# arkworks-rs/pcd

Measured on AMD Instinct MI355X. Metric: msm_mscalar_mul_per_s, higher is better.
Workload: dtype u32 (11 x 28-bit unsaturated Montgomery limbs, v_mad_u64_u32 with 64-bit column accumulators); 1 GPU; MNT4-298 G1 variable-base MSM, n=1048576 pairs per GPU (2^20 per GPU), proving-key bases and scalars resident in HBM, scalar distribution uniform; curve=MNT4-298, group=G1, log_n=20, window_bits=20, windows=15

## Files before the change

pcd_amd/csrc/msm.hip.h:

```cpp
#pragma once
#include <cstdlib>
#include <math.h>

#include <algorithm>
#include <type_traits>
#include <vector>

#include "ec.hip.h"

namespace pcd {

template <int K>
struct EventSet {
  hipEvent_t e[K] = {};
  bool live = false;
  hipError_t create() {
    for (int i = 0; i < K; i++) { hipError_t r = hipEventCreate(&e[i]); if (r != hipSuccess) return r; }
    live = true;
    return hipSuccess;
  }
  hipEvent_t operator[](int i) const { return e[i]; }
  ~EventSet() { for (int i = 0; i < K; i++) if (e[i]) (void)hipEventDestroy(e[i]); }
};

// ... 254 lines not shown
  off[(size_t)b * KB + 2 * t] = ex;
  off[(size_t)b * KB + 2 * t + 1] = ex + c0;
  __syncthreads();
  for (uint32_t p0 = lo + threadIdx.x; p0 < hi; p0 += MSM_SORT_UNROLL * blockDim.x) {
    uint64_t e[MSM_SORT_UNROLL];
    uint32_t pos[MSM_SORT_UNROLL];
#pragma unroll
    for (int u = 0; u < MSM_SORT_UNROLL; u++) { uint32_t p = p0 + u * blockDim.x; e[u] = p < hi ? entries[p] : ~0ull; }
#pragma unroll
    for (int u = 0; u < MSM_SORT_UNROLL; u++) if (e[u] != ~0ull) pos[u] = atomicAdd(&hist[(uint32_t)(e[u] >> 32) & (KB - 1)], 1u);
#pragma unroll
    for (int u = 0; u < MSM_SORT_UNROLL; u++) if (e[u] != ~0ull) sorted_idx[pos[u]] = (uint32_t)e[u];
  }
}

static __global__ void __launch_bounds__(1024) scan_block_sums(const uint32_t* __restrict__ in, uint32_t n, uint32_t per_block,
                                                         uint32_t* __restrict__ block_sums) {
  __shared__ uint32_t sh[1024];
  uint32_t b = blockIdx.x, lo = b * per_block, hi = min(n, lo + per_block);
  uint32_t acc = 0;
  for (uint32_t i = lo + threadIdx.x; i < hi; i += blockDim.x) acc += in[i];
  sh[threadIdx.x] = acc;
  __syncthreads();
  for (int s = 512; s > 0; s >>= 1) { if ((int)threadIdx.x < s) sh[threadIdx.x] += sh[threadIdx.x + s]; __syncthreads(); }
  if (threadIdx.x == 0) block_sums[b] = sh[0];
}
static __global__ void __launch_bounds__(1024) scan_apply(const uint32_t* __restrict__ in, uint32_t n, uint32_t per_block,
                                                    const uint32_t* __restrict__ block_sums, uint32_t nblocks,
                                                    uint32_t* __restrict__ out ) {
  __shared__ uint32_t sh[1024];
  __shared__ uint32_t carry;
  uint32_t b = blockIdx.x, lo = b * per_block, hi = min(n, lo + per_block);
  if (threadIdx.x == 0) { uint32_t a = 0; for (uint32_t k = 0; k < b; k++) a += block_sums[k]; carry = a; }
  __syncthreads();
  for (uint32_t base = lo; base < hi; base += 1024) {
    uint32_t i = base + threadIdx.x;
    uint32_t v = (i < hi) ? in[i] : 0;
    sh[threadIdx.x] = v;
    __syncthreads();
    for (int s = 1; s < 1024; s <<= 1) {
      uint32_t t = ((int)threadIdx.x >= s) ? sh[threadIdx.x - s] : 0;
      __syncthreads();
      sh[threadIdx.x] += t;
      __syncthreads();
    }
    if (i < hi) out[i] = carry + sh[threadIdx.x] - v;
    __syncthreads();
    if (threadIdx.x == 0) carry += sh[1023];
    __syncthreads();
  }
  if (b == nblocks - 1 && threadIdx.x == 0) out[n] = carry;
}

PCD_HD uint32_t msm_plan_chunk(uint32_t M, uint32_t lanes, uint32_t lo, uint32_t hi) {
  const uint64_t per_round = (uint64_t)lanes * hi;
  const uint64_t rounds = ((uint64_t)M + per_round - 1) / per_round;
  const uint32_t chunk = rounds ? (uint32_t)(((uint64_t)M + (uint64_t)lanes * rounds - 1) / ((uint64_t)lanes * rounds)) : lo;
  return chunk < lo ? lo : chunk > hi ? hi : chunk;
}
PCD_HD uint32_t msm_plan_word(uint32_t lanes, uint32_t lo, uint32_t hi) { return lanes | (lo << 20) | (hi << 26); }
PCD_HD uint32_t msm_chunk_of_plan(uint32_t M, uint32_t plan) { return msm_plan_chunk(M, plan & 0xFFFFFu, (plan >> 20) & 63u, (plan >> 26) & 63u); }

PCD_DEV uint32_t msm_find_key(const uint32_t* __restrict__ off, uint32_t nkeys, uint32_t p) {
  uint32_t lo = 0, hi = nkeys;
  while (hi - lo > 1) { uint32_t mid = (lo + hi) >> 1; if (off[mid] <= p) lo = mid; else hi = mid; }
  return lo;
}

struct MsmEntrySource {
  const uint32_t* sorted_idx;
  const uint32_t* slots;
  const uint32_t* ones_idx;
  const uint32_t* flag;
  uint32_t cap, ones_key;
};
struct MsmCursor {
  uint32_t key, key_start, key_end;
  uint32_t next_end;
  PCD_DEV void seek(const uint32_t* __restrict__ off, uint32_t nkeys, uint32_t p) {
    key = msm_find_key(off, nkeys, p);
    key_start = off[key];
    key_end = off[key + 1];
    next_end = key + 2 <= nkeys ? off[key + 2] : key_end;
  }
  PCD_DEV void advance_to(const uint32_t* __restrict__ off, uint32_t nkeys, uint32_t p) {
    for (int step = 0; step < 4 && p >= key_end; step++) {
      key++; key_start = key_end; key_end = next_end;
      next_end = key + 2 <= nkeys ? off[key + 2] : key_end;
    }
    if (p >= key_end) seek(off, nkeys, p);
  }
};
PCD_DEV uint32_t msm_entry(const MsmEntrySource& src, bool compact, const MsmCursor& cur, uint32_t p) {
  if (cur.key == src.ones_key) return compact && !src.ones_idx ? src.sorted_idx[p] : src.ones_idx[p - cur.key_start];
  return compact ? src.sorted_idx[p] : src.slots[(size_t)cur.key * src.cap + (p - cur.key_start)];
}

#ifndef PCD_BASE_ALIGN
#define PCD_BASE_ALIGN 1
#endif
template <class G>
struct MsmBaseStride {
  static constexpr int W = Aff<typename G::F>::WORDS;
  static constexpr int value = (PCD_BASE_ALIGN && W == 22) ? 32 : W;
};

template <class G>
struct MsmUseXyzz {
  typedef typename G::F F;
#ifndef PCD_XYZZ_753
#define PCD_XYZZ_753 0
#endif
  static constexpr bool value = F::Base::INLINE_ARITH || F::DEG == 2 || (PCD_XYZZ_753 && F::Base::N > 11);
};
// ... 89 lines not shown
    typename EC<G>::AccX a = {F::load(p), F::load(p + F::WORDS), F::load(p + 2 * F::WORDS), F::load(p + 3 * F::WORDS)};
    return EC<G>::x_to_jac(a);
  }
  static constexpr bool SEPARATE = true;
};
template <class G>
struct MsmStoredPlain<G, false> {
  typedef typename G::F F;
  static constexpr int WORDS = Jac<F>::WORDS;
  PCD_DEV static Jac<F> load(const uint32_t* p) { return Jac<F>::load(p); }
  static constexpr bool SEPARATE = false;
};
template <class G, bool LAZY = LazyCapable<typename G::F>::value>
struct MsmStored : MsmStoredPlain<G> {};
template <class G>
struct MsmStored<G, true> {
  typedef typename G::F F;
  static constexpr int WORDS = EC<G>::ACC_WORDS;
  PCD_DEV static Jac<F> load(const uint32_t* p) {
    typename EC<G>::AccLz a;
    a.ZZ = F::load(p + 2 * F::WORDS);
    if (a.ZZ.is_zero()) return Jac<F>::infinity();
    a.inf = false;
#pragma unroll
    for (int i = 0; i < F::N; i++) a.X.v[i] = (int32_t)p[i];
    a.Y = F::load(p + F::WORDS);
    a.ZZZ = F::load(p + 3 * F::WORDS);
    return EC<G>::lz_to_jac(a);
  }
  static constexpr bool SEPARATE = true;
};

template <class G>
struct MsmAccWaves {
  typedef typename AccOf<G>::type::F FA;
#ifndef PCD_ACC_WAVES_SPLIT
#define PCD_ACC_WAVES_SPLIT 2
#endif
#ifndef PCD_ACC_WAVES_G1
#define PCD_ACC_WAVES_G1 2
#endif
#ifndef PCD_ACC_WAVES_MB298
#define PCD_ACC_WAVES_MB298 2
#endif
  static constexpr int value = !FA::Base::INLINE_ARITH ? (FA::Base::N <= 11 ? PCD_ACC_WAVES_MB298 : 1)
                             : FA::DEG == 1 ? PCD_ACC_WAVES_G1 : AccOf<G>::LANES > 1 ? PCD_ACC_WAVES_SPLIT : 1;
};

template <class G, bool COMPACT>
__global__ void __launch_bounds__(64, MsmAccWaves<G>::value) msm_accumulate_kernel(const uint32_t* __restrict__ bases, const MsmEntrySource src,
                                                            const uint32_t* __restrict__ off, uint32_t nkeys,
                                                            uint32_t chunk, uint32_t* __restrict__ buckets,
                                                            uint32_t* __restrict__ piece_first, uint32_t* __restrict__ piece_last,
                                                            uint32_t plan ) {
  if (plan) chunk = msm_chunk_of_plan(off[nkeys], plan);
  typedef typename AccOf<G>::type GA;
  typedef typename GA::F F;
  typedef EC<GA> E;
  constexpr int RW = MsmStored<GA>::WORDS;
  constexpr uint32_t LANES = AccOf<G>::LANES, PER_WAVE = 64 / LANES;
  if (threadIdx.x >= PER_WAVE * LANES) return;
  uint32_t t = blockIdx.x * PER_WAVE + threadIdx.x / LANES;
  const uint32_t M = off[nkeys];
  uint64_t start64 = (uint64_t)t * chunk;
  if (start64 >= M) return;
  uint32_t start = (uint32_t)start64, end = (uint32_t)min((uint64_t)M, start64 + chunk);
  if (!COMPACT && src.flag && *src.flag != 0) return;
  if (COMPACT && src.flag && *src.flag == 0) return;
  MsmCursor cur;
  cur.seek(off, nkeys, start);
  bool open_start = cur.key_start < start;
#if PCD_ACC_LDS
  typename std::conditional<LazyCapable<F>::value, MsmRunLazyLds<GA>, MsmRunPlain<GA>>::type acc;
#else
  typename std::conditional<LazyCapable<F>::value, MsmRunLazy<GA>, MsmRunPlain<GA>>::type acc;
#endif
  constexpr bool PREFETCH = F::Base::INLINE_ARITH;
  const uint32_t ones_start = off[src.ones_key];
  auto point_of = [&](uint32_t e) {
    Aff<F> q = Aff<F>::load(bases + (size_t)(e & ~MSM_NEG) * MsmBaseStride<G>::value);
    const F ny = q.y.neg();
    if (e & MSM_NEG) q.y = ny;
    return q;
  };
  if constexpr (COMPACT) {
    auto entry_at = [&](uint32_t pos) { return (src.ones_idx && pos >= ones_start) ? src.ones_idx[pos - ones_start] : src.sorted_idx[pos]; };
    Aff<F> nxt;
    if (PREFETCH) nxt = point_of(entry_at(start));
    for (uint32_t p = start; p < end; p++) {
      if (p >= cur.key_end) {
        if (open_start) { acc.flush(piece_first + (size_t)t * RW); open_start = false; }
        else acc.flush(buckets + (size_t)cur.key * RW);
        cur.advance_to(off, nkeys, p);
      }
      if (PREFETCH) {
        const Aff<F> pt = nxt;
        if (p + 1 < end) nxt = point_of(entry_at(p + 1));
        acc.add(pt);
      } else {
        acc.add(point_of(entry_at(p)));
      }
    }
  } else {
    MsmCursor nxt_cur = cur;
    Aff<F> nxt;
    if (PREFETCH) nxt = point_of(msm_entry(src, false, cur, start));
    for (uint32_t p = start; p < end; p++) {
// ... 259 lines not shown
      MsmRunPlain<GA> acc;
      uint32_t key = key_first;
      for (uint32_t i = 0; i < cnt; i++) {
        const uint32_t k0 = in[(size_t)(2 * i) * 64], l0 = in[(size_t)(2 * i + 1) * 64];
        if (k0 != key) {
          if (open_start) { acc.flush(piece_first + (size_t)t * RW); open_start = false; }
          else acc.flush(buckets + (size_t)key * RW);
          key = k0;
        }
        acc.add(point_of(l0));
      }
      const bool open_end = off[key + 1] > end;
      if (open_end) acc.flush(piece_last + (size_t)t * RW);
      else if (open_start) acc.flush(piece_first + (size_t)t * RW);
      else acc.flush(buckets + (size_t)key * RW);
    }
  }
}

template <class G>
struct MsmItems {
  typedef typename SplitOfTail<G>::type GA;
  static constexpr uint32_t LANES = SplitOfTail<G>::LANES, PER_WAVE = 64 / LANES;
  PCD_DEV static bool idle() { return threadIdx.x >= PER_WAVE * LANES; }
  PCD_DEV static uint32_t local() { return threadIdx.x / LANES; }
  PCD_DEV static uint32_t item() { return blockIdx.x * PER_WAVE + threadIdx.x / LANES; }
  static uint32_t grid(uint32_t items) { return (items + PER_WAVE - 1) / PER_WAVE; }
};

static __global__ void __launch_bounds__(256) msm_zero_kernel(uint32_t* __restrict__ cnt, uint32_t n_cnt, uint32_t* __restrict__ ctl4) {
  const uint32_t i = blockIdx.x * blockDim.x + threadIdx.x;
  if (i < n_cnt) cnt[i] = 0;
  if (i < 4) ctl4[i] = 0;
}

#ifndef PCD_SINGLE_ITEM_PLAIN
#define PCD_SINGLE_ITEM_PLAIN 0
#endif
template <class G> struct MsmSingleItem {
  typedef typename std::conditional<PCD_SINGLE_ITEM_PLAIN != 0, typename SplitOf<G>::type, typename SplitOfTail<G>::type>::type GA;
  static constexpr int LANES = PCD_SINGLE_ITEM_PLAIN != 0 ? SplitOf<G>::LANES : SplitOfTail<G>::LANES;
};
template <class G>
__global__ void __launch_bounds__(64) msm_merge_ones_kernel(uint32_t* __restrict__ buckets, uint32_t ones_key) {
  typedef typename MsmSingleItem<G>::GA GA;
  typedef typename GA::F F;
  if (blockIdx.x != 0 || threadIdx.x >= MsmSingleItem<G>::LANES) return;
  Jac<F> a = Jac<F>::load(buckets + (size_t)1 * Jac<F>::WORDS);
  Jac<F> b = Jac<F>::load(buckets + (size_t)ones_key * Jac<F>::WORDS);
  EC<GA>::add(a, b).store(buckets + (size_t)1 * Jac<F>::WORDS);
}

template <class G>
__global__ void __launch_bounds__(64) msm_fixup_kernel(const uint32_t* __restrict__ off, uint32_t nkeys, uint32_t chunk,
                                                       const uint32_t* __restrict__ piece_first, const uint32_t* __restrict__ piece_last,
                                                       const uint32_t* __restrict__ acc_buckets ,
                                                       uint32_t* __restrict__ buckets, uint32_t big_limit, uint32_t* __restrict__ big_count,
                                                       uint32_t* __restrict__ big_list , uint32_t big_cap,
                                                       uint32_t* __restrict__ seg_list , uint32_t seg_len,
                                                       const uint32_t* __restrict__ chunk_dev ,
                                                       uint32_t plan ) {
  if (chunk_dev) chunk = *chunk_dev;
  else if (plan) chunk = msm_chunk_of_plan(off[nkeys], plan);
  typedef typename MsmItems<G>::GA GA;
  typedef typename GA::F F;
  typedef EC<GA> E;
  constexpr int RW = MsmStored<GA>::WORDS;
  if (MsmItems<G>::idle()) return;
  const bool lead = threadIdx.x % MsmItems<G>::LANES == 0;
  uint32_t key = MsmItems<G>::item();
  if (key >= nkeys) return;
  uint32_t lo = off[key], hi = off[key + 1];
  if (hi == lo) {
    F::zero().store(buckets + (size_t)key * Jac<F>::WORDS + 2 * F::WORDS);
    return;
  }
  uint32_t t0 = lo / chunk, t1 = (hi - 1) / chunk;
  if (t1 == t0) {
    if (MsmStored<GA>::SEPARATE) MsmStored<GA>::load(acc_buckets + (size_t)key * RW).store(buckets + (size_t)key * Jac<F>::WORDS);
    return;
  }
  if (t1 - t0 + 1 > big_limit) {
    if (!lead) return;
    uint32_t nseg = (t1 - t0 + seg_len) / seg_len;
    uint32_t slot = atomicAdd(&big_count[0], 1u);
    uint32_t s0 = atomicAdd(&big_count[1], nseg);
    if (slot < big_cap) { big_list[3 * slot] = key; big_list[3 * slot + 1] = s0; big_list[3 * slot + 2] = nseg; }
    for (uint32_t i = 0; i < nseg; i++) {
      uint32_t lo = t0 + i * seg_len, hi = min(t1, lo + seg_len - 1);
      seg_list[3 * (s0 + i)] = lo; seg_list[3 * (s0 + i) + 1] = hi; seg_list[3 * (s0 + i) + 2] = t1;
    }
    return;
  }
  Jac<F> acc = MsmStored<GA>::load(piece_last + (size_t)t0 * RW);
  for (uint32_t u = t0 + 1; u < t1; u++) acc = E::add(acc, MsmStored<GA>::load(piece_last + (size_t)u * RW));
  acc = E::add(acc, MsmStored<GA>::load(piece_first + (size_t)t1 * RW));
  acc.store(buckets + (size_t)key * Jac<F>::WORDS);
}

template <class G, bool ENABLE = true, bool Q = true>
struct MsmPairItems {
  static constexpr bool TWO = ENABLE && TwoLaneOps<G>::value && (MsmItems<G>::LANES == 1 || HalfLanes<typename MsmItems<G>::GA::F>::L == (int)MsmItems<G>::LANES);
  static constexpr bool QUAD = Q && TWO && MsmItems<G>::LANES == 1 && PCD_EC4 != 0;
  static constexpr uint32_t BASE = MsmItems<G>::LANES, LANES = QUAD ? 4 : TWO ? 2 * BASE : BASE, PER_WAVE = 64 / LANES;
  PCD_DEV static bool idle() { return threadIdx.x >= PER_WAVE * LANES; }
  PCD_DEV static uint32_t item() { return blockIdx.x * PER_WAVE + threadIdx.x / LANES; }
  PCD_DEV static uint32_t local() { return threadIdx.x / LANES; }
  PCD_DEV static bool writer() { return QUAD ? (threadIdx.x & 3u) == 0 : (!TWO || (((threadIdx.x & 63u) / BASE) & 1u) == 0); }
  static uint32_t grid(uint32_t items) { return (items + PER_WAVE - 1) / PER_WAVE; }
};
template <class G, bool TWO = MsmPairItems<G, true>::TWO, bool Q = true>
struct MsmPairOps {
  typedef typename MsmItems<G>::GA GA;
  typedef Jac<typename GA::F> J;
  PCD_DEV static J add(const J& a, const J& b) { return EC<GA>::add(a, b); }
  PCD_DEV static J dbl(const J& a) { return EC<GA>::dbl(a); }
};
template <class G, bool Q>
struct MsmPairOps<G, true, Q> {
  typedef typename SplitOfTail<G>::type GA;
  typedef Jac<typename GA::F> J;
  PCD_DEV static J add(const J& a, const J& b) { if constexpr (MsmPairItems<G, true, Q>::QUAD) return EC4<GA>::add4(a, b); else return EC2<GA>::add2(a, b); }
  PCD_DEV static J dbl(const J& a) { if constexpr (MsmPairItems<G, true, Q>::QUAD) return EC4<GA>::dbl4(a); else return EC2<GA>::dbl2(a); }
};
template <class G>
PCD_DEV void msm_wave_tree(Jac<typename MsmPairOps<G>::GA::F> acc, uint32_t* my , uint32_t* dst) {
  typedef MsmPairItems<G> IT;
  typedef MsmPairOps<G> O;
  typedef typename O::GA::F F;
  constexpr uint32_t PW = IT::PER_WAVE;
  const uint32_t it = IT::local();
  const bool live = !IT::idle();
  if (live && IT::writer()) acc.store(my + (size_t)it * Jac<F>::WORDS);
  __syncthreads();
  for (uint32_t s = 32; s > 0; s >>= 1) {
    if (live && it < s && it + s < PW) {
      Jac<F> o = Jac<F>::load(my + (size_t)(it + s) * Jac<F>::WORDS);
      acc = O::add(acc, o);
      if (IT::writer()) acc.store(my + (size_t)it * Jac<F>::WORDS);
    }
    __syncthreads();
  }
  if (live && it == 0 && IT::writer()) acc.store(dst);
  __syncthreads();
}
template <class G>
__global__ void __launch_bounds__(64) msm_big_segments_kernel(const uint32_t* __restrict__ seg_list, const uint32_t* __restrict__ big_count,
                                                              const uint32_t* __restrict__ piece_first, const uint32_t* __restrict__ piece_last,
                                                              uint32_t* __restrict__ partial, uint32_t* __restrict__ scratch) {
  typedef MsmPairItems<G> IT;
  typedef MsmPairOps<G> O;
  typedef typename O::GA GA;
  typedef typename GA::F F;
  constexpr uint32_t PW = IT::PER_WAVE;
  const uint32_t nseg = big_count[1];
  uint32_t* my = scratch + (size_t)blockIdx.x * 64 * Jac<F>::WORDS;
  for (uint32_t sg = blockIdx.x; sg < nseg; sg += gridDim.x) {
    uint32_t lo = seg_list[3 * sg], hi = seg_list[3 * sg + 1], tlast = seg_list[3 * sg + 2];
    Jac<F> acc = Jac<F>::infinity();
    if (!IT::idle())
      for (uint32_t u = lo + IT::local(); u <= hi; u += PW) {
        const uint32_t* src = (u == tlast) ? piece_first : piece_last;
        acc = O::add(acc, MsmStored<GA>::load(src + (size_t)u * MsmStored<GA>::WORDS));
      }
    msm_wave_tree<G>(acc, my, partial + (size_t)sg * Jac<F>::WORDS);
  }
}
template <class G>
__global__ void __launch_bounds__(64) msm_big_bucket_kernel(const uint32_t* __restrict__ big_list, const uint32_t* __restrict__ big_count,
                                                            const uint32_t* __restrict__ partial, uint32_t* __restrict__ buckets,
                                                            uint32_t* __restrict__ scratch) {
  typedef MsmPairItems<G> IT;
  typedef MsmPairOps<G> O;
  typedef typename O::GA GA;
  typedef typename GA::F F;
  constexpr uint32_t PW = IT::PER_WAVE;
  const uint32_t nbig = big_count[0];
  uint32_t* my = scratch + (size_t)blockIdx.x * 64 * Jac<F>::WORDS;
  for (uint32_t b = blockIdx.x; b < nbig; b += gridDim.x) {
    uint32_t key = big_list[3 * b], s0 = big_list[3 * b + 1], ns = big_list[3 * b + 2];
    Jac<F> acc = Jac<F>::infinity();
    if (!IT::idle())
      for (uint32_t u = IT::local(); u < ns; u += PW) acc = O::add(acc, Jac<F>::load(partial + (size_t)(s0 + u) * Jac<F>::WORDS));
    msm_wave_tree<G>(acc, my, buckets + (size_t)key * Jac<F>::WORDS);
  }
}

template <class G, bool WIDE>
__global__ void __launch_bounds__(64) msm_tail_level_kernel(const uint32_t* __restrict__ A_in, uint32_t mA, size_t strideA_in,
                                                            const uint32_t* __restrict__ C_in, uint32_t mC, size_t strideC_in,
                                                            uint32_t* __restrict__ A_out, size_t strideA_out,
                                                            uint32_t* __restrict__ C_out, size_t strideC_out, int k) {
  typedef MsmPairItems<G, WIDE> IT;
  typedef MsmPairOps<G, IT::TWO> O;
  typedef typename O::GA GA;
  typedef typename GA::F F;
  constexpr int PW = Jac<F>::WORDS;
  if (IT::idle()) return;
  uint32_t K = 1u << k;
  uint32_t JA = (mA + K - 1) >> k, JC = (mC + K - 1) >> k;
  uint32_t tid = IT::item();
  uint32_t w = blockIdx.y;
  if (tid < JA) {
    const uint32_t* A = A_in + w * strideA_in * PW;
    Jac<F> run = Jac<F>::infinity(), acc = Jac<F>::infinity();
    for (int tt = (int)K - 1; tt >= 0; tt--) {
      uint32_t i = tid * K + tt;
      if (i < mA) run = O::add(run, Jac<F>::load(A + (size_t)i * PW));
      acc = O::add(acc, run);
    }
    if (IT::writer()) acc.store(C_out + (w * strideC_out + JC + tid) * PW);
    if (tid >= 1) {
      for (int d = 0; d < k; d++) run = O::dbl(run);
      if (IT::writer()) run.store(A_out + (w * strideA_out + tid - 1) * PW);
    }
  } else if (tid < JA + JC) {
    uint32_t j = tid - JA;
    const uint32_t* Cw = C_in + w * strideC_in * PW;
    Jac<F> acc = Jac<F>::infinity();
    for (uint32_t tt = 0; tt < K; tt++) {
      uint32_t i = j * K + tt;
      if (i < mC) acc = O::add(acc, Jac<F>::load(Cw + (size_t)i * PW));
    }
    if (IT::writer()) acc.store(C_out + (w * strideC_out + j) * PW);
  }
}

template <class G, bool Q = true>
PCD_DEV void msm_tail_pair_item(int role, uint32_t j, uint32_t w, const uint32_t* A_in, uint32_t mA, size_t strideA_in, const uint32_t* C_in,
                                uint32_t mC, size_t strideC_in, uint32_t* A_out, size_t strideA_out, uint32_t* C_out, size_t strideC_out) {
  typedef MsmPairOps<G, MsmPairItems<G, true>::TWO, Q> O;
  typedef typename O::GA GA;
  typedef typename GA::F F;
  typedef MsmPairItems<G, true, Q> IT;
  constexpr int PW = Jac<F>::WORDS;
  const uint32_t JA = (mA + 1) >> 1, JC = (mC + 1) >> 1;
  if (role < 2) {
    if (j >= JA) return;
    const uint32_t* A = A_in + w * strideA_in * PW;
    const bool two = 2 * j + 1 < mA;
    const Jac<F> a0 = Jac<F>::load(A + (size_t)(2 * j) * PW);
    if (role == 0) {
      if (j == 0) return;
      Jac<F> run = two ? O::add(a0, Jac<F>::load(A + (size_t)(2 * j + 1) * PW)) : a0;
      run = O::dbl(run);
      if (IT::writer()) run.store(A_out + (w * strideA_out + j - 1) * PW);
    } else {
      Jac<F> acc = two ? O::add(O::dbl(Jac<F>::load(A + (size_t)(2 * j + 1) * PW)), a0) : a0;
      if (IT::writer()) acc.store(C_out + (w * strideC_out + JC + j) * PW);
    }
  } else {
    if (j >= JC) return;
    const uint32_t* Cw = C_in + w * strideC_in * PW;
    Jac<F> acc = Jac<F>::load(Cw + (size_t)(2 * j) * PW);
    if (2 * j + 1 < mC) acc = O::add(acc, Jac<F>::load(Cw + (size_t)(2 * j + 1) * PW));
    if (IT::writer()) acc.store(C_out + (w * strideC_out + j) * PW);
  }
}
template <class G, bool Q = true>
__global__ void __launch_bounds__(64) msm_tail_pair_kernel(const uint32_t* __restrict__ A_in, uint32_t mA, size_t strideA_in,
                                                           const uint32_t* __restrict__ C_in, uint32_t mC, size_t strideC_in,
                                                           uint32_t* __restrict__ A_out, size_t strideA_out,
                                                           uint32_t* __restrict__ C_out, size_t strideC_out) {
  typedef MsmPairItems<G, true, Q> IT;
  if (IT::idle()) return;
  msm_tail_pair_item<G, Q>((int)blockIdx.z, IT::item(), blockIdx.y, A_in, mA, strideA_in, C_in, mC, strideC_in, A_out, strideA_out, C_out, strideC_out);
}
constexpr uint32_t MSM_FUSED_WAVES = 4;
#ifndef PCD_QUAD_MAX_ITEMS
#define PCD_QUAD_MAX_ITEMS 4096
#endif
constexpr uint32_t MSM_QUAD_MAX_ITEMS = PCD_QUAD_MAX_ITEMS;
template <class G>
struct MsmFusedTail {
  static constexpr bool ENABLED = !MsmPairOps<G>::GA::F::Base::MAILBOX;
  static uint32_t waves(uint32_t items) { return (items + MsmPairItems<G>::PER_WAVE - 1) / MsmPairItems<G>::PER_WAVE; }
  static bool fits(uint32_t mA, uint32_t mC) { return ENABLED && 2 * waves((mA + 1) >> 1) + waves((mC + 1) >> 1) <= MSM_FUSED_WAVES; }
};
template <class G>
__global__ void __launch_bounds__(64 * MSM_FUSED_WAVES) msm_tail_fused_kernel(const uint32_t* A_in, uint32_t mA, size_t strideA_in, const uint32_t* C_in,
                                                                              uint32_t mC, size_t strideC_in, uint32_t* A0, uint32_t* A1, uint32_t* C0,
                                                                              uint32_t* C1, size_t strideAC, int flip) {
  typedef MsmPairItems<G> IT;
  const uint32_t wave = threadIdx.x >> 6, lane = threadIdx.x & 63u;
  const bool idle = lane >= IT::PER_WAVE * IT::LANES;
  const uint32_t w = blockIdx.x;
  while (mA > 0 || mC > 1) {
    const uint32_t JA = (mA + 1) >> 1, JC = (mC + 1) >> 1;
    uint32_t* A_out = flip ? A1 : A0;
    uint32_t* C_out = flip ? C1 : C0;
    const uint32_t wa = (JA + IT::PER_WAVE - 1) / IT::PER_WAVE;
    const int role = wave < wa ? 0 : wave < 2 * wa ? 1 : 2;
    const uint32_t j = (wave - (uint32_t)role * wa) * IT::PER_WAVE + lane / IT::LANES;
    if (!idle) msm_tail_pair_item<G>(role, j, w, A_in, mA, strideA_in, C_in, mC, strideC_in, A_out, strideAC, C_out, strideAC);
    __syncthreads();
    mA = JA ? JA - 1 : 0;
    mC = JC + JA;
    A_in = A_out; strideA_in = strideAC;
    C_in = C_out; strideC_in = strideAC;
    flip ^= 1;
  }
}

template <class G>
__global__ void __launch_bounds__(64) msm_horner_kernel(const uint32_t* __restrict__ C, size_t strideC, int W, int c, uint32_t* __restrict__ out) {
  typedef typename MsmSingleItem<G>::GA GA;
  typedef typename GA::F F;
  typedef EC<GA> E;
  constexpr int PW = Jac<F>::WORDS;
  if (blockIdx.x != 0 || threadIdx.x >= MsmSingleItem<G>::LANES) return;
  Jac<F> total = Jac<F>::load(C + (size_t)(W - 1) * strideC * PW);
  for (int w = W - 2; w >= 0; w--) {
    for (int d = 0; d < c; d++) total = E::dbl(total);
    total = E::add(total, Jac<F>::load(C + (size_t)w * strideC * PW));
  }
  total.store(out);
}

template <class G>
// ... 123 lines not shown
struct MsmSharedSort {
  bool valid = false;
  uint32_t n = 0, n_total = 0, offset = 0, tkeys = 0;
  int c = 0, W = 0, groups = 0;
  const uint32_t* scalars = nullptr;
  const uint32_t* inf_bits = nullptr;
  MsmEntrySource src{};
  const uint32_t* off = nullptr;
  hipEvent_t ready = nullptr;
};
enum { MSM_SHARE_NONE = 0, MSM_SHARE_PRODUCE = 1, MSM_SHARE_CONSUME = 2 };

template <class G>
hipError_t msm_run(MsmWorkspace& ws, hipStream_t st, const MsmBasesView& bv, const uint32_t* scalars_dev, uint32_t n,
                   uint32_t* out_dev, int c_override, uint32_t chunk_override, int sort_mode, MsmTimings* tm,
                   MsmSharedSort* share = nullptr, int share_role = MSM_SHARE_NONE) {
  const int acc_mode = (sort_mode >> 4) & 3;
  const uint32_t tree_chunk = ((uint32_t)sort_mode >> 8) & 0xFFFu, tree_min_pairs = ((uint32_t)sort_mode >> 20) & 0xFFu;
  sort_mode &= 15;
  const bool single_pass = sort_mode == 1;
  const uint32_t* bases_dev = bv.dptr;
  typedef typename G::F F;
  constexpr int NS = G::FR::N32;
  constexpr int PW = Jac<F>::WORDS;
  constexpr size_t PB = (size_t)PW * 4;
  if (n == 0) { ws.last_err_dev = nullptr; Jac<F> inf = Jac<F>::infinity(); return hipMemcpyAsync(out_dev, &inf, PB, hipMemcpyHostToDevice, st); }
  MsmPlan pl;
  pl.n = n;
  pl.c = bv.groups > 1 ? bv.c : (c_override ? c_override : msm_pick_window(n, G::FR::BITS, 0));
  pl.W = msm_num_windows(G::FR::BITS, pl.c);
  const int Wg = (pl.W + bv.groups - 1) / bv.groups;
  pl.nkeys = (uint32_t)Wg << pl.c;
  const uint64_t maxM = (uint64_t)n * pl.W;
  pl.chunk = chunk_override ? chunk_override : 40;
  int& cus = ws.cus;
  if (!cus) {
    int dev = 0;
    if (hipGetDevice(&dev) != hipSuccess || hipDeviceGetAttribute(&cus, hipDeviceAttributeMultiprocessorCount, dev) != hipSuccess || cus <= 0) cus = 256;
  }
  bool use_tree = false;
  uint32_t tree_cap = 0;
  const uint32_t* tree_chunk_dev = nullptr;
  if constexpr (MsmTreeCapable<G>::value) {
    use_tree = acc_mode == 2 && (uint64_t)bv.n_total * bv.groups < MSM_SCR;
    if (use_tree) {
      tree_cap = tree_chunk ? tree_chunk : MSM_TREE_CHUNK_MAX;
      pl.chunk = tree_cap;
    }
  }
  const MsmLane* lane = ws.lane;
  const int plan_cus = lane && lane->cus > 0 ? lane->cus : cus;
  uint32_t acc_lanes = 0, chunk_lo = 0;
  static const uint32_t chunk_hi_env = getenv("PCDHIP_CHUNK_HI") ? (uint32_t)atoi(getenv("PCDHIP_CHUNK_HI")) : 0u;
  const uint32_t chunk_hi = chunk_hi_env >= 16 && chunk_hi_env <= 63 ? chunk_hi_env : 56;
  if (!chunk_override && !use_tree) {
    acc_lanes = (uint32_t)plan_cus * 4 * MsmAccWaves<G>::value * (64 / AccOf<G>::LANES);
    chunk_lo = (uint32_t)std::min<uint64_t>(40, std::max<uint64_t>(16, (maxM + 4ull * acc_lanes - 1) / (4ull * acc_lanes)));
    pl.chunk = chunk_lo;
  }
  const uint32_t plan_word = acc_lanes && acc_lanes < (1u << 20) && chunk_hi < 64 ? msm_plan_word(acc_lanes, chunk_lo, chunk_hi) : 0u;
  if (acc_lanes && !plan_word) pl.chunk = 40;
  if (maxM >= 0xFFFFFFF0ull || (uint64_t)bv.n_total * bv.groups >= 0x7FFFFFF0ull) return hipErrorInvalidValue;

  EventSet<9> ev;
  if (tm) PCD_HIP_TRY(ev.create());
  auto mark = [&](int i) -> hipError_t { return tm ? hipEventRecord(ev[i], st) : hipSuccess; };

  const uint32_t tkeys = pl.nkeys + 1, ones_key = pl.nkeys;
  const bool consume = share && share_role == MSM_SHARE_CONSUME && share->valid && share->n == n && share->n_total == bv.n_total &&
                       share->offset == bv.offset && share->tkeys == tkeys && share->c == pl.c && share->W == pl.W &&
                       share->groups == bv.groups && share->scalars == scalars_dev &&
                       (share->inf_bits == nullptr || share->inf_bits == bv.inf_bits);
  PCD_HIP_TRY(ws.ensure(WS_CNT, (size_t)tkeys * 4 + 16));
  PCD_HIP_TRY(ws.ensure(WS_OFF, ((size_t)tkeys + 1) * 4));
  const uint32_t scan_per_block = 16384;
  const uint32_t scan_blocks = (tkeys + scan_per_block - 1) / scan_per_block;
  PCD_HIP_TRY(ws.ensure(WS_BSUM, (size_t)scan_blocks * 4));
  PCD_HIP_TRY(ws.ensure(WS_SORTED, (size_t)maxM * 4));
  PCD_HIP_TRY(ws.ensure(WS_BUCKETS, (size_t)tkeys * PB));
  PCD_HIP_TRY(ws.ensure(WS_OUT, PB + 64));
  PCD_HIP_TRY(ws.ensure(WS_ONES, (size_t)n * 4 + 32));
  uint32_t* cnt = (uint32_t*)ws.buf[WS_CNT];
  uint32_t* off = (uint32_t*)ws.buf[WS_OFF];
  uint32_t* bsum = (uint32_t*)ws.buf[WS_BSUM];
  uint32_t* sorted = (uint32_t*)ws.buf[WS_SORTED];
  uint32_t* buckets = (uint32_t*)ws.buf[WS_BUCKETS];
  uint32_t* ones_idx = (uint32_t*)ws.buf[WS_ONES];
  uint32_t* flag = ones_idx + n;
  uint32_t* err = flag + 1;
  uint32_t* big_count = flag + 2;
  auto zero_start = [&](uint32_t n_cnt) {
    hipLaunchKernelGGL(msm_zero_kernel, dim3(std::max<uint32_t>(1u, (n_cnt + 255) / 256)), dim3(256), 0, st, cnt, n_cnt, flag);
  };
  ws.last_err_dev = consume ? nullptr : err;
  constexpr int SBITS = G::FR::BITS;
  const int wins = (pl.W + Wg - 1) / Wg;
  const int top_bits = G::FR::BITS + 1 - (pl.W - 1) * pl.c;
  double mu = (double)n * wins / (double)(1u << (pl.c - 1)) + (top_bits < pl.c ? (double)n / (double)(1u << top_bits) : 0.0);
  uint32_t cap = (uint32_t)(mu + 6.0 * sqrt(mu) + 8.0);
  cap = (cap + 7u) & ~7u;
  const bool use_slots = single_pass && (double)pl.nkeys * cap * 4.0 <= 1.5e9;
  const uint32_t nbins = pl.nkeys >> MSM_BIN_SHIFT;
  const bool use_partition = sort_mode == 0 && pl.c >= MSM_BIN_SHIFT && nbins >= 1 && nbins <= MSM_MAX_BINS && n >= 4096;
  uint32_t* slots = nullptr;
  if (use_slots) { PCD_HIP_TRY(ws.ensure(WS_SLOTS, (size_t)pl.nkeys * cap * 4)); slots = (uint32_t*)ws.buf[WS_SLOTS]; }

  PCD_HIP_TRY(mark(0));
  dim3 gd((n + 255) / 256), bd(256);
  MsmEntrySource src;
  if (consume) {
    PCD_HIP_TRY(hipStreamWaitEvent(st, share->ready, 0));
    zero_start(0);
    src = share->src;
// ... 71 lines not shown
  const uint32_t seg_cap = nchunks / seg_len + big_cap + 2;
  PCD_HIP_TRY(ws.ensure(WS_BIG, (size_t)(3 * big_cap + 3 * seg_cap + 8) * 4));
  PCD_HIP_TRY(ws.ensure(WS_BIGPART, (size_t)seg_cap * PB));
  uint32_t* pfirst = (uint32_t*)ws.buf[WS_PFIRST];
  uint32_t* plast = (uint32_t*)ws.buf[WS_PLAST];
  uint32_t* big = (uint32_t*)ws.buf[WS_BIG];
  uint32_t* seg_list = big + 3 * big_cap;
  uint32_t* big_partial = (uint32_t*)ws.buf[WS_BIGPART];
  PCD_HIP_TRY(mark(8));
  hipStream_t own = st;
  if (lane) {
    if (!ws.lane_in) PCD_HIP_TRY(hipEventCreateWithFlags(&ws.lane_in, hipEventDisableTiming));
    if (!ws.lane_out) PCD_HIP_TRY(hipEventCreateWithFlags(&ws.lane_out, hipEventDisableTiming));
    PCD_HIP_TRY(hipEventRecord(ws.lane_in, own));
    PCD_HIP_TRY(hipStreamWaitEvent(lane->stream, ws.lane_in, 0));
    st = lane->stream;
  }
  {
    constexpr uint32_t per_wave = 64 / AccOf<G>::LANES;
    const dim3 acc_grid((nchunks + per_wave - 1) / per_wave);
    bool launched = false;
    if constexpr (MsmTreeCapable<G>::value) {
      if (use_tree) {
        constexpr int FW = AccOf<G>::type::F::WORDS;
        const uint32_t grid = tree_grid;
        MsmTreeBufs tb;
        tb.cap = tree_cap;
        tb.phases = 3;
        uint32_t* chunk_word = big_count + 2;
        hipLaunchKernelGGL(msm_tree_plan_kernel, dim3(1), dim3(1), 0, st, off, tkeys, grid * 64, tree_cap, tree_chunk, chunk_word);
        tree_chunk_dev = chunk_word;
        PCD_HIP_TRY(ws.ensure(WS_TLIST, MsmTreeBufs::list_words(tb.cap) * 4 * grid));
        PCD_HIP_TRY(ws.ensure(WS_TPAIR, MsmTreeBufs::pair_words(tb.cap) * 4 * grid));
        PCD_HIP_TRY(ws.ensure(WS_TPREFIX, MsmTreeBufs::prefix_words(tb.cap, FW) * 4 * grid));
        PCD_HIP_TRY(ws.ensure(WS_TPTS, MsmTreeBufs::pts_words(tb.cap, FW) * 4 * grid));
        tb.list = (uint32_t*)ws.buf[WS_TLIST]; tb.pairs = (uint32_t*)ws.buf[WS_TPAIR];
        tb.prefix = (uint32_t*)ws.buf[WS_TPREFIX]; tb.pts = (uint32_t*)ws.buf[WS_TPTS];
        hipLaunchKernelGGL((msm_pair_tree_kernel<G>), dim3(grid), dim3(64), 0, st, bases_dev, src, off, tkeys, chunk_word, tb,
                           tree_min_pairs ? tree_min_pairs : MSM_TREE_MIN_PAIRS, acc_buckets, pfirst, plast);
        launched = true;
      }
    }
    if (!launched) {
      if (src.slots) hipLaunchKernelGGL((msm_accumulate_kernel<G, false>), acc_grid, dim3(64), 0, st, bases_dev, src, off, tkeys, pl.chunk, acc_buckets, pfirst, plast, plan_word);
      hipLaunchKernelGGL((msm_accumulate_kernel<G, true>), acc_grid, dim3(64), 0, st, bases_dev, src, off, tkeys, pl.chunk, acc_buckets, pfirst, plast, plan_word);
    }
  }
  if (lane) {
    PCD_HIP_TRY(hipEventRecord(ws.lane_out, st));
    st = own;
    PCD_HIP_TRY(hipStreamWaitEvent(st, ws.lane_out, 0));
  }
  PCD_HIP_TRY(mark(4));
  hipLaunchKernelGGL((msm_fixup_kernel<G>), dim3(MsmItems<G>::grid(tkeys)), dim3(64), 0, st, off, tkeys, pl.chunk, pfirst, plast, acc_buckets, buckets,
                     big_limit, big_count, big, big_cap, seg_list, seg_len, tree_chunk_dev, plan_word);
  {
    const uint32_t big_grid = std::min<uint32_t>(seg_cap, 2048);
    PCD_HIP_TRY(ws.ensure(WS_BIGSCR, (size_t)big_grid * 64 * PB));
    hipLaunchKernelGGL((msm_big_segments_kernel<G>), dim3(big_grid), dim3(64), 0, st, seg_list, big_count, pfirst, plast, big_partial,
                       (uint32_t*)ws.buf[WS_BIGSCR]);
    hipLaunchKernelGGL((msm_big_bucket_kernel<G>), dim3(std::min<uint32_t>(big_cap, 2048)), dim3(64), 0, st, big, big_count, big_partial,
                       buckets, (uint32_t*)ws.buf[WS_BIGSCR]);
  }
  hipLaunchKernelGGL((msm_merge_ones_kernel<G>), dim3(1), dim3(64), 0, st, buckets, ones_key);
  PCD_HIP_TRY(mark(5));
  {
    const uint32_t B = 1u << (pl.c - 1);
    size_t cap_pts = ((size_t)1 << pl.c);
    PCD_HIP_TRY(ws.ensure(WS_A0, (size_t)Wg * cap_pts * PB / 2 + PB * Wg * 4));
    PCD_HIP_TRY(ws.ensure(WS_A1, (size_t)Wg * cap_pts * PB / 2 + PB * Wg * 4));
    PCD_HIP_TRY(ws.ensure(WS_C0, (size_t)Wg * cap_pts * PB / 2 + PB * Wg * 4));
    PCD_HIP_TRY(ws.ensure(WS_C1, (size_t)Wg * cap_pts * PB / 2 + PB * Wg * 4));
    const size_t strideAC = cap_pts / 2 + 4;
    const uint32_t* A_in = buckets + PW;
    size_t strideA_in = (size_t)1 << pl.c;
    const uint32_t* C_in = nullptr;
    size_t strideC_in = 0;
    uint32_t mA = B, mC = 0;
    int flip = 0, level = 0;
    bool fused = false;
    while (mA > 0 || mC > 1) {
      int k = (level == 0 && B >= (1u << 17)) ? 3 : 1;
      uint32_t K = 1u << k;
      uint32_t JA = (mA + K - 1) >> k, JC = (mC + K - 1) >> k;
      uint32_t* A_out = (uint32_t*)ws.buf[flip ? WS_A1 : WS_A0];
      uint32_t* C_out = (uint32_t*)ws.buf[flip ? WS_C1 : WS_C0];
      uint32_t threads = JA + JC;
      if (!fused && level > 0 && MsmFusedTail<G>::fits(mA, mC)) {
        hipLaunchKernelGGL((msm_tail_fused_kernel<G>), dim3(Wg), dim3(64 * MSM_FUSED_WAVES), 0, st, A_in, mA, strideA_in, C_in, mC, strideC_in,
                           (uint32_t*)ws.buf[WS_A0], (uint32_t*)ws.buf[WS_A1], (uint32_t*)ws.buf[WS_C0], (uint32_t*)ws.buf[WS_C1], strideAC, flip);
        fused = true;
      }
      if (fused) {
      } else if (k == 1 && std::max(JA, JC) * (uint32_t)Wg > MSM_QUAD_MAX_ITEMS)
        hipLaunchKernelGGL((msm_tail_pair_kernel<G, false>), dim3(MsmPairItems<G, true, false>::grid(std::max(JA, JC)), Wg, 3), dim3(64), 0, st, A_in, mA,
                           strideA_in, C_in, mC, strideC_in, A_out, strideAC, C_out, strideAC);
      else if (k == 1)
        hipLaunchKernelGGL((msm_tail_pair_kernel<G>), dim3(MsmPairItems<G>::grid(std::max(JA, JC)), Wg, 3), dim3(64), 0, st, A_in, mA, strideA_in, C_in,
                           mC, strideC_in, A_out, strideAC, C_out, strideAC);
      else if (threads <= (1u << 15))
        hipLaunchKernelGGL((msm_tail_level_kernel<G, true>), dim3(MsmPairItems<G, true>::grid(threads), Wg), dim3(64), 0, st, A_in, mA, strideA_in, C_in, mC,
                           strideC_in, A_out, strideAC, C_out, strideAC, k);
      else
        hipLaunchKernelGGL((msm_tail_level_kernel<G, false>), dim3(MsmPairItems<G, false>::grid(threads), Wg), dim3(64), 0, st, A_in, mA, strideA_in, C_in, mC,
                           strideC_in, A_out, strideAC, C_out, strideAC, k);
      mA = JA ? JA - 1 : 0;
      mC = JC + JA;
      A_in = A_out; strideA_in = strideAC;
      C_in = C_out; strideC_in = strideAC;
      flip ^= 1;
      level++;
    }
    PCD_HIP_TRY(mark(6));
    hipLaunchKernelGGL((msm_horner_kernel<G>), dim3(1), dim3(64), 0, st, C_in, strideC_in, Wg, pl.c, out_dev);
    PCD_HIP_TRY(mark(7));
  }
  PCD_HIP_TRY(hipGetLastError());
  if (tm) {
    PCD_HIP_TRY(hipStreamSynchronize(st));
    auto el = [&](int a, int b) { float ms = 0; (void)hipEventElapsedTime(&ms, ev[a], ev[b]); return ms; };
    tm->digits = el(0, 1); tm->scan = el(1, 2); tm->scatter = el(2, 8); tm->accumulate = el(8, 4);
    tm->fixup = el(4, 5); tm->tail = el(5, 6); tm->horner = el(6, 7); tm->total = el(0, 7);
    PCD_HIP_TRY(hipMemcpy(&tm->entries, off + tkeys, 4, hipMemcpyDeviceToHost));
    tm->chunk = plan_word ? msm_chunk_of_plan(tm->entries, plan_word) : pl.chunk;
    if (tree_chunk_dev) PCD_HIP_TRY(hipMemcpy(&tm->chunk, tree_chunk_dev, 4, hipMemcpyDeviceToHost));
  }
  return hipSuccess;
}

}
```

Measured before the change: 391.2 Mscalar-mul/s.

## Fix up only chunk-spanning buckets and read single-chunk buckets directly in tail

The fixup kernel now launches one item per accumulate chunk boundary, plus two special keys, instead of one item per bucket key. It binary-searches the key that straddles each boundary and merges only those pieces. The first tail reduction level reads buckets that fit in one chunk straight from the accumulate output, instead of relying on fixup to copy every bucket into the final bucket array. This removes a full per-bucket copy pass and shrinks the fixup grid. In exchange, the first tail level does extra offset lookups and branches per bucket. The plan word is widened to 64 bits so the maximum chunk size can exceed 63.

```diff
diff --git a/pcd_amd/csrc/msm.hip.h b/pcd_amd/csrc/msm.hip.h
--- a/pcd_amd/csrc/msm.hip.h
+++ b/pcd_amd/csrc/msm.hip.h
@@ -330,14 +330,32 @@
   if (b == nblocks - 1 && threadIdx.x == 0) out[n] = carry;
 }
 
+PCD_HD uint64_t msm_plan_rounds(uint32_t M, uint32_t lanes, uint32_t hi) {
+  const uint64_t per_round = (uint64_t)lanes * hi;
+  return ((uint64_t)M + per_round - 1) / per_round;
+}
 PCD_HD uint32_t msm_plan_chunk(uint32_t M, uint32_t lanes, uint32_t lo, uint32_t hi) {
-  const uint64_t per_round = (uint64_t)lanes * hi;
-  const uint64_t rounds = ((uint64_t)M + per_round - 1) / per_round;
+  const uint64_t rounds = msm_plan_rounds(M, lanes, hi);
   const uint32_t chunk = rounds ? (uint32_t)(((uint64_t)M + (uint64_t)lanes * rounds - 1) / ((uint64_t)lanes * rounds)) : lo;
   return chunk < lo ? lo : chunk > hi ? hi : chunk;
 }
-PCD_HD uint32_t msm_plan_word(uint32_t lanes, uint32_t lo, uint32_t hi) { return lanes | (lo << 20) | (hi << 26); }
-PCD_HD uint32_t msm_chunk_of_plan(uint32_t M, uint32_t plan) { return msm_plan_chunk(M, plan & 0xFFFFFu, (plan >> 20) & 63u, (plan >> 26) & 63u); }
+constexpr uint32_t MSM_CHUNK_MAX = 128;
+#ifndef PCD_CHUNK_HI
+#define PCD_CHUNK_HI 56
+#endif
+constexpr uint32_t MSM_CHUNK_HI = PCD_CHUNK_HI;
+PCD_HD uint64_t msm_plan_word(uint32_t lanes, uint32_t lo, uint32_t hi) { return (uint64_t)lanes | ((uint64_t)lo << 20) | ((uint64_t)hi << 28); }
+PCD_HD uint32_t msm_chunk_of_plan(uint32_t M, uint64_t plan) {
+  return msm_plan_chunk(M, (uint32_t)(plan & 0xFFFFFu), (uint32_t)(plan >> 20) & 255u, (uint32_t)(plan >> 28) & 255u);
+}
+struct MsmChunkRule {
+  const uint32_t* chunk_dev;
+  uint64_t plan;
+  uint32_t chunk;
+  PCD_DEV uint32_t eval(const uint32_t* __restrict__ off, uint32_t nkeys) const {
+    return chunk_dev ? *chunk_dev : plan ? msm_chunk_of_plan(off[nkeys], plan) : chunk;
+  }
+};
 
 PCD_DEV uint32_t msm_find_key(const uint32_t* __restrict__ off, uint32_t nkeys, uint32_t p) {
   uint32_t lo = 0, hi = nkeys;
@@ -533,7 +551,7 @@
                                                             const uint32_t* __restrict__ off, uint32_t nkeys,
                                                             uint32_t chunk, uint32_t* __restrict__ buckets,
                                                             uint32_t* __restrict__ piece_first, uint32_t* __restrict__ piece_last,
-                                                            uint32_t plan ) {
+                                                            uint64_t plan ) {
   if (plan) chunk = msm_chunk_of_plan(off[nkeys], plan);
   typedef typename AccOf<G>::type GA;
   typedef typename GA::F F;
@@ -899,34 +917,35 @@
 }
 
 template <class G>
-__global__ void __launch_bounds__(64) msm_fixup_kernel(const uint32_t* __restrict__ off, uint32_t nkeys, uint32_t chunk,
+__global__ void __launch_bounds__(64) msm_fixup_kernel(const uint32_t* __restrict__ off, uint32_t nkeys, const MsmChunkRule rule,
                                                        const uint32_t* __restrict__ piece_first, const uint32_t* __restrict__ piece_last,
                                                        const uint32_t* __restrict__ acc_buckets ,
                                                        uint32_t* __restrict__ buckets, uint32_t big_limit, uint32_t* __restrict__ big_count,
                                                        uint32_t* __restrict__ big_list , uint32_t big_cap,
-                                                       uint32_t* __restrict__ seg_list , uint32_t seg_len,
-                                                       const uint32_t* __restrict__ chunk_dev ,
-                                                       uint32_t plan ) {
-  if (chunk_dev) chunk = *chunk_dev;
-  else if (plan) chunk = msm_chunk_of_plan(off[nkeys], plan);
+                                                       uint32_t* __restrict__ seg_list , uint32_t seg_len) {
+  const uint32_t chunk = rule.eval(off, nkeys);
   typedef typename MsmItems<G>::GA GA;
   typedef typename GA::F F;
   typedef EC<GA> E;
   constexpr int RW = MsmStored<GA>::WORDS;
   if (MsmItems<G>::idle()) return;
   const bool lead = threadIdx.x % MsmItems<G>::LANES == 0;
-  uint32_t key = MsmItems<G>::item();
-  if (key >= nkeys) return;
-  uint32_t lo = off[key], hi = off[key + 1];
-  if (hi == lo) {
-    F::zero().store(buckets + (size_t)key * Jac<F>::WORDS + 2 * F::WORDS);
+  const uint32_t item = MsmItems<G>::item();
+  if (item < 2) {
+    const uint32_t key = item == 0 ? 1u : nkeys - 1;
+    const uint32_t lo = off[key], hi = off[key + 1];
+    if (hi == lo) F::zero().store(buckets + (size_t)key * Jac<F>::WORDS + 2 * F::WORDS);
+    else if (MsmStored<GA>::SEPARATE && hi - (lo / chunk) * chunk <= chunk)
+      MsmStored<GA>::load(acc_buckets + (size_t)key * RW).store(buckets + (size_t)key * Jac<F>::WORDS);
     return;
   }
-  uint32_t t0 = lo / chunk, t1 = (hi - 1) / chunk;
-  if (t1 == t0) {
-    if (MsmStored<GA>::SEPARATE) MsmStored<GA>::load(acc_buckets + (size_t)key * RW).store(buckets + (size_t)key * Jac<F>::WORDS);
-    return;
-  }
+  const uint32_t t0 = item - 2;
+  const uint64_t edge = ((uint64_t)t0 + 1) * chunk;
+  if (edge >= off[nkeys]) return;
+  const uint32_t key = msm_find_key(off, nkeys, (uint32_t)edge - 1);
+  const uint32_t lo = off[key], hi = off[key + 1];
+  if (hi <= (uint32_t)edge || lo / chunk != t0) return;
+  const uint32_t t1 = (hi - 1) / chunk;
   if (t1 - t0 + 1 > big_limit) {
     if (!lead) return;
     uint32_t nseg = (t1 - t0 + seg_len) / seg_len;
@@ -1033,8 +1052,26 @@
   }
 }
 
+struct MsmBucketSrc {
+  const uint32_t* off;
+  const uint32_t* acc_buckets;
+  const uint32_t* buckets;
+  uint32_t nkeys;
+  MsmChunkRule rule;
+};
+template <class GA>
+PCD_DEV Jac<typename GA::F> msm_bucket_at(const MsmBucketSrc& bs, uint32_t chunk, uint32_t key) {
+  typedef typename GA::F F;
+  if (key != 1) {
+    const uint32_t lo = bs.off[key], hi = bs.off[key + 1];
+    if (hi == lo) return Jac<F>::infinity();
+    if (hi - (lo / chunk) * chunk <= chunk)
+      return MsmStored<GA>::load(bs.acc_buckets + (size_t)key * MsmStored<GA>::WORDS);
+  }
+  return Jac<F>::load(bs.buckets + (size_t)key * Jac<F>::WORDS);
+}
 template <class G, bool WIDE>
-__global__ void __launch_bounds__(64) msm_tail_level_kernel(const uint32_t* __restrict__ A_in, uint32_t mA, size_t strideA_in,
+__global__ void __launch_bounds__(64) msm_tail_level_kernel(const MsmBucketSrc bs, uint32_t mA, size_t strideA_in,
                                                             const uint32_t* __restrict__ C_in, uint32_t mC, size_t strideC_in,
                                                             uint32_t* __restrict__ A_out, size_t strideA_out,
                                                             uint32_t* __restrict__ C_out, size_t strideC_out, int k) {
@@ -1049,11 +1086,12 @@
   uint32_t tid = IT::item();
   uint32_t w = blockIdx.y;
   if (tid < JA) {
-    const uint32_t* A = A_in + w * strideA_in * PW;
+    const uint32_t chunk = bs.rule.eval(bs.off, bs.nkeys);
+    const uint32_t key1 = w * (uint32_t)strideA_in + 1;
     Jac<F> run = Jac<F>::infinity(), acc = Jac<F>::infinity();
     for (int tt = (int)K - 1; tt >= 0; tt--) {
       uint32_t i = tid * K + tt;
-      if (i < mA) run = O::add(run, Jac<F>::load(A + (size_t)i * PW));
+      if (i < mA) run = O::add(run, msm_bucket_at<GA>(bs, chunk, key1 + i));
       acc = O::add(acc, run);
     }
     if (IT::writer()) acc.store(C_out + (w * strideC_out + JC + tid) * PW);
@@ -1073,9 +1111,10 @@
   }
 }
 
-template <class G, bool Q = true>
+template <class G, bool Q = true, bool FIRST = false>
 PCD_DEV void msm_tail_pair_item(int role, uint32_t j, uint32_t w, const uint32_t* A_in, uint32_t mA, size_t strideA_in, const uint32_t* C_in,
-                                uint32_t mC, size_t strideC_in, uint32_t* A_out, size_t strideA_out, uint32_t* C_out, size_t strideC_out) {
+                                uint32_t mC, size_t strideC_in, uint32_t* A_out, size_t strideA_out, uint32_t* C_out, size_t strideC_out,
+                                const MsmBucketSrc* bs = nullptr) {
   typedef MsmPairOps<G, MsmPairItems<G, true>::TWO, Q> O;
   typedef typename O::GA GA;
   typedef typename GA::F F;
@@ -1084,16 +1123,21 @@
   const uint32_t JA = (mA + 1) >> 1, JC = (mC + 1) >> 1;
   if (role < 2) {
     if (j >= JA) return;
-    const uint32_t* A = A_in + w * strideA_in * PW;
+    uint32_t chunk = 0;
+    if constexpr (FIRST) chunk = bs->rule.eval(bs->off, bs->nkeys);
+    auto a_at = [&](uint32_t i) {
+      if constexpr (FIRST) return msm_bucket_at<GA>(*bs, chunk, w * (uint32_t)strideA_in + 1 + i);
+      else return Jac<F>::load(A_in + (w * strideA_in + i) * PW);
+    };
     const bool two = 2 * j + 1 < mA;
-    const Jac<F> a0 = Jac<F>::load(A + (size_t)(2 * j) * PW);
+    const Jac<F> a0 = a_at(2 * j);
     if (role == 0) {
       if (j == 0) return;
-      Jac<F> run = two ? O::add(a0, Jac<F>::load(A + (size_t)(2 * j + 1) * PW)) : a0;
+      Jac<F> run = two ? O::add(a0, a_at(2 * j + 1)) : a0;
       run = O::dbl(run);
       if (IT::writer()) run.store(A_out + (w * strideA_out + j - 1) * PW);
     } else {
-      Jac<F> acc = two ? O::add(O::dbl(Jac<F>::load(A + (size_t)(2 * j + 1) * PW)), a0) : a0;
+      Jac<F> acc = two ? O::add(O::dbl(a_at(2 * j + 1)), a0) : a0;
       if (IT::writer()) acc.store(C_out + (w * strideC_out + JC + j) * PW);
     }
   } else {
@@ -1112,6 +1156,14 @@
   typedef MsmPairItems<G, true, Q> IT;
   if (IT::idle()) return;
   msm_tail_pair_item<G, Q>((int)blockIdx.z, IT::item(), blockIdx.y, A_in, mA, strideA_in, C_in, mC, strideC_in, A_out, strideA_out, C_out, strideC_out);
+}
+template <class G, bool Q = true>
+__global__ void __launch_bounds__(64) msm_tail_pair_first_kernel(const MsmBucketSrc bs, uint32_t mA, size_t strideA_in,
+                                                                 uint32_t* __restrict__ A_out, size_t strideA_out,
+                                                                 uint32_t* __restrict__ C_out, size_t strideC_out) {
+  typedef MsmPairItems<G, true, Q> IT;
+  if (IT::idle()) return;
+  msm_tail_pair_item<G, Q, true>((int)blockIdx.z, IT::item(), blockIdx.y, nullptr, mA, strideA_in, nullptr, 0u, 0, A_out, strideA_out, C_out, strideC_out, &bs);
 }
 constexpr uint32_t MSM_FUSED_WAVES = 4;
 #ifndef PCD_QUAD_MAX_ITEMS
@@ -1341,13 +1393,13 @@
   const int plan_cus = lane && lane->cus > 0 ? lane->cus : cus;
   uint32_t acc_lanes = 0, chunk_lo = 0;
   static const uint32_t chunk_hi_env = getenv("PCDHIP_CHUNK_HI") ? (uint32_t)atoi(getenv("PCDHIP_CHUNK_HI")) : 0u;
-  const uint32_t chunk_hi = chunk_hi_env >= 16 && chunk_hi_env <= 63 ? chunk_hi_env : 56;
+  const uint32_t chunk_hi = chunk_hi_env >= 16 && chunk_hi_env <= MSM_CHUNK_MAX ? chunk_hi_env : MSM_CHUNK_HI;
   if (!chunk_override && !use_tree) {
     acc_lanes = (uint32_t)plan_cus * 4 * MsmAccWaves<G>::value * (64 / AccOf<G>::LANES);
     chunk_lo = (uint32_t)std::min<uint64_t>(40, std::max<uint64_t>(16, (maxM + 4ull * acc_lanes - 1) / (4ull * acc_lanes)));
     pl.chunk = chunk_lo;
   }
-  const uint32_t plan_word = acc_lanes && acc_lanes < (1u << 20) && chunk_hi < 64 ? msm_plan_word(acc_lanes, chunk_lo, chunk_hi) : 0u;
+  const uint64_t plan_word = acc_lanes && acc_lanes < (1u << 20) ? msm_plan_word(acc_lanes, chunk_lo, chunk_hi) : 0u;
   if (acc_lanes && !plan_word) pl.chunk = 40;
   if (maxM >= 0xFFFFFFF0ull || (uint64_t)bv.n_total * bv.groups >= 0x7FFFFFF0ull) return hipErrorInvalidValue;
 
@@ -1525,8 +1577,9 @@
     PCD_HIP_TRY(hipStreamWaitEvent(st, ws.lane_out, 0));
   }
   PCD_HIP_TRY(mark(4));
-  hipLaunchKernelGGL((msm_fixup_kernel<G>), dim3(MsmItems<G>::grid(tkeys)), dim3(64), 0, st, off, tkeys, pl.chunk, pfirst, plast, acc_buckets, buckets,
-                     big_limit, big_count, big, big_cap, seg_list, seg_len, tree_chunk_dev, plan_word);
+  const MsmChunkRule chunk_rule = {tree_chunk_dev, plan_word, pl.chunk};
+  hipLaunchKernelGGL((msm_fixup_kernel<G>), dim3(MsmItems<G>::grid(nchunks + 2)), dim3(64), 0, st, off, tkeys, chunk_rule, pfirst, plast, acc_buckets,
+                     buckets, big_limit, big_count, big, big_cap, seg_list, seg_len);
   {
     const uint32_t big_grid = std::min<uint32_t>(seg_cap, 2048);
     PCD_HIP_TRY(ws.ensure(WS_BIGSCR, (size_t)big_grid * 64 * PB));
@@ -1545,6 +1598,7 @@
     PCD_HIP_TRY(ws.ensure(WS_C0, (size_t)Wg * cap_pts * PB / 2 + PB * Wg * 4));
     PCD_HIP_TRY(ws.ensure(WS_C1, (size_t)Wg * cap_pts * PB / 2 + PB * Wg * 4));
     const size_t strideAC = cap_pts / 2 + 4;
+    const MsmBucketSrc bucket_src = {off, acc_buckets, buckets, tkeys, chunk_rule};
     const uint32_t* A_in = buckets + PW;
     size_t strideA_in = (size_t)1 << pl.c;
     const uint32_t* C_in = nullptr;
@@ -1565,18 +1619,24 @@
         fused = true;
       }
       if (fused) {
-      } else if (k == 1 && std::max(JA, JC) * (uint32_t)Wg > MSM_QUAD_MAX_ITEMS)
+      } else if (level == 0 && k == 1 && JA * (uint32_t)Wg > MSM_QUAD_MAX_ITEMS)
+        hipLaunchKernelGGL((msm_tail_pair_first_kernel<G, false>), dim3(MsmPairItems<G, true, false>::grid(JA), Wg, 2), dim3(64), 0, st, bucket_src, mA,
+                           strideA_in, A_out, strideAC, C_out, strideAC);
+      else if (level == 0 && k == 1)
+        hipLaunchKernelGGL((msm_tail_pair_first_kernel<G>), dim3(MsmPairItems<G>::grid(JA), Wg, 2), dim3(64), 0, st, bucket_src, mA, strideA_in, A_out,
+                           strideAC, C_out, strideAC);
+      else if (k == 1 && std::max(JA, JC) * (uint32_t)Wg > MSM_QUAD_MAX_ITEMS)
         hipLaunchKernelGGL((msm_tail_pair_kernel<G, false>), dim3(MsmPairItems<G, true, false>::grid(std::max(JA, JC)), Wg, 3), dim3(64), 0, st, A_in, mA,
                            strideA_in, C_in, mC, strideC_in, A_out, strideAC, C_out, strideAC);
       else if (k == 1)
         hipLaunchKernelGGL((msm_tail_pair_kernel<G>), dim3(MsmPairItems<G>::grid(std::max(JA, JC)), Wg, 3), dim3(64), 0, st, A_in, mA, strideA_in, C_in,
                            mC, strideC_in, A_out, strideAC, C_out, strideAC);
       else if (threads <= (1u << 15))
-        hipLaunchKernelGGL((msm_tail_level_kernel<G, true>), dim3(MsmPairItems<G, true>::grid(threads), Wg), dim3(64), 0, st, A_in, mA, strideA_in, C_in, mC,
-                           strideC_in, A_out, strideAC, C_out, strideAC, k);
+        hipLaunchKernelGGL((msm_tail_level_kernel<G, true>), dim3(MsmPairItems<G, true>::grid(threads), Wg), dim3(64), 0, st, bucket_src, mA, strideA_in, C_in,
+                           mC, strideC_in, A_out, strideAC, C_out, strideAC, k);
       else
-        hipLaunchKernelGGL((msm_tail_level_kernel<G, false>), dim3(MsmPairItems<G, false>::grid(threads), Wg), dim3(64), 0, st, A_in, mA, strideA_in, C_in, mC,
-                           strideC_in, A_out, strideAC, C_out, strideAC, k);
+        hipLaunchKernelGGL((msm_tail_level_kernel<G, false>), dim3(MsmPairItems<G, false>::grid(threads), Wg), dim3(64), 0, st, bucket_src, mA, strideA_in, C_in,
+                           mC, strideC_in, A_out, strideAC, C_out, strideAC, k);
       mA = JA ? JA - 1 : 0;
       mC = JC + JA;
       A_in = A_out; strideA_in = strideAC;
```

Result: no change. 398.4 Mscalar-mul/s, median of 6 (+1.8%).
